# XuyangBai/PointDSC

Measured on AMD Instinct MI355X. Metric: point-cloud pairs/sec @ N=5000 corr, higher is better.
Workload: dtype f32 (attention products as fp16x3 split (fp16 hi+lo operand pairs, three f16 MFMAs per product), f32 accumulate; fc_message / PointCN products as fp16 hi+lo split; spatial-consistency matrix stored as unorm16); 1 GPU; 3DMatch-like synthetic correspondences (BASELINE.json configs[2]): N=5000 corr, 32 pairs per step sharded over 1 GPU(s) = 32 per GPU, 12-layer PointDSC, seeded random weights; num_corr=5000, pairs_per_gpu=32, global_batch=32, compat_format=u16, layer_gemm=h3, att_leaves=canonical, latency_mode=False, range_guard=lazy (pipeline), collective=none (single process, no process group)

## Files before the change

include/pointdsc_hip.h:

```cpp
#ifndef POINTDSC_HIP_H
#define POINTDSC_HIP_H

#include <stddef.h>

#ifdef __cplusplus
extern "C" {
#endif

#define PDSC_VERSION 9
#define PDSC_CHANNELS 128
#define PDSC_MAX_K 64
#define PDSC_MAX_POWER_ITERS 32

enum pdsc_status {
    PDSC_OK = 0,
    PDSC_ERR_ARG = -1,
    PDSC_ERR_WORKSPACE = -2,
    PDSC_ERR_LAUNCH = -3
};

typedef struct pdsc_config {
    int in_dim;
    int num_layers;
    int num_channels;
// ... 98 lines not shown
    float* featB_out;
    float* qkv_out;
    void* q_split;
    void* kv_tiles;
    const void* w1; const float* b1;
    const void* w2; const float* b2;
    const void* w3; const float* b3;
    const void* wp; const float* bp;
    const void* wq; const float* bq;
    const void* wq_split;
    const void* wfrag_tail;
    const void* wfrag_head;
    int gemm_format;
    int io_flags;
    int bs, N;
    int kernel;
} pdsc_layer_call;
int pdsc_layer_run(const pdsc_layer_call* call, void* stream);

size_t    pdsc_wsplit_bytes(const pdsc_config* cfg);
long long pdsc_wsplit_offset(const pdsc_config* cfg, int section, int layer);
int       pdsc_wsplit_build(const pdsc_config* cfg, const float* wpack, void* wsplit, void* stream);
#define PDSC_WS_FRAG_TAIL 100
#define PDSC_WS_FRAG_HEAD 101
#define PDSC_WS_FRAG_TAIL_H3 102
#define PDSC_WS_FRAG_HEAD_H3 103
#define PDSC_WS_FOLD_TAIL_H3 104
#define PDSC_WS_FOLD_HEAD_H3 105
#define PDSC_WS_FOLD_W 106
size_t pdsc_wfrag_fold_tail_bytes(void);
size_t pdsc_wfrag_fold_head_bytes(void);
int pdsc_layer_prefers_block(int bs, int N);
int pdsc_layer_h3_uses_coop(int bs, int N);
size_t pdsc_wfrag_tail_bytes(void);
size_t pdsc_wfrag_head_bytes(void);
int pdsc_wfrag_build_tail(const float* w1, const float* b1, const float* w2, const float* b2, const float* w3,
                          const float* b3, void* out, int gemm_format, void* stream);
int pdsc_wfrag_build_head(const float* wp, const float* bp, const float* wq, const float* bq, void* out,
                          int gemm_format, void* stream);

size_t pdsc_attention_scratch_bytes(int bs, int N, int nsplit);
int    pdsc_attention_default_split(int bs, int N);
int    pdsc_sc_attention(const float* qkv, const float* compat, long long ld, float* msg,
                         void* scratch, size_t scratch_bytes, int bs, int N, int nsplit, void* stream);

size_t pdsc_split_q_bytes(int bs, int N);
size_t pdsc_split_kv_bytes(int bs, int N);
int    pdsc_pack_qkv_split(const float* qkv, void* q_split, void* kv_tiles, int bs, int N, void* stream);
size_t pdsc_attention_split_scratch_bytes(int bs, int N, int nsplit);
int    pdsc_attention_split_default_split(int bs, int N);
int    pdsc_attention_leaf_count(int N);
int    pdsc_attention_leaf_plan(int bs, int N, int leaves_mode, int* nsplit, int* nleaf);
size_t pdsc_attention_leaf_scratch_bytes(int bs, int N, int leaves_mode);
int    pdsc_sc_attention_split(const void* q_split, const void* kv_tiles, const float* compat, long long ld,
                               float* msg, void* scratch, size_t scratch_bytes, int bs, int N, int nsplit,
                               void* stream);
int    pdsc_sc_attention_split_u16(const void* q_split, const void* kv_tiles, const unsigned short* compat_u16, long long ld,
                                   float* msg, void* scratch, size_t scratch_bytes, int bs, int N, int nsplit,
                                   void* stream);

int pdsc_attention_trace(long long* device_buffer);

int pdsc_layer_trace(long long* device_buffer);

int pdsc_classifier_hidden(const float* feat, const float* W1, const float* b1, const float* W2, const float* b2, float* h2,
                           int M, void* stream);
// ... 174 lines not shown
```

pointdsc_amd/_lib.py:

```python
from __future__ import annotations

import ctypes as C
import os
from pathlib import Path

PKG = Path(__file__).resolve().parent
LIB_PATH = Path(os.environ.get("POINTDSC_HIP_LIB", PKG / "libpointdsc_hip.so"))


class PointDSCLibraryError(RuntimeError):
    pass


class PdscConfig(C.Structure):
    _fields_ = [
        ("in_dim", C.c_int), ("num_layers", C.c_int), ("num_channels", C.c_int),
        ("num_iterations", C.c_int), ("k", C.c_int), ("refine_iters", C.c_int),
        ("inlier_threshold", C.c_float), ("nms_radius", C.c_float), ("refine_threshold", C.c_float),
        ("attention_precision", C.c_int), ("compat_format", C.c_int), ("layer_gemm", C.c_int),
        ("att_leaves", C.c_int), ("value_fold", C.c_int),
    ]


W_SECTIONS = [
# ... 6 lines not shown
_cfgp = C.POINTER(PdscConfig)


class PdscLayerCall(C.Structure):
    _fields_ = (
        [(n, _vp) for n in ("msg", "part_o", "part_ml")] + [("nsplit", _i), ("Npad", _i)] +
        [(n, _vp) for n in ("res", "feat_in", "feat_out", "featB_out", "qkv_out", "q_split", "kv_tiles",
                            "w1", "b1", "w2", "b2", "w3", "b3", "wp", "bp", "wq", "bq", "wq_split", "wfrag_tail", "wfrag_head")] +
        [(n, _i) for n in ("gemm_format", "io_flags", "bs", "N", "kernel")])

SIGNATURES = {
    "pdsc_version": (_i, []),
    "pdsc_set_range_report": (_i, [_vp]),
    "pdsc_last_error": (C.c_char_p, []),
    "pdsc_experiments_enabled": (_i, []),
    "pdsc_wpack_floats": (_ll, [_cfgp]),
    "pdsc_wpack_offset": (_ll, [_cfgp, _i, _i]),
    "pdsc_compat_ld": (_ll, [_i]),
    "pdsc_workspace_bytes": (_sz, [_cfgp, _i, _i, _i]),
    "pdsc_workspace_offset": (_ll, [_cfgp, _i, _i, _i, C.c_char_p]),
    "pdsc_spatial_compat": (_i, [_vp, _vp, _vp, _vp, _vp, _ll, _i, _i, _vp]),
    "pdsc_spatial_compat_u16": (_i, [_vp, _vp, _vp, _vp, _ll, _i, _i, _vp]),
    "pdsc_selftest_exact_math": (_i, [_vp, _f, _vp, _vp, _ll, _vp]),
    "pdsc_selftest_mfma_valu_neighbour": (_i, [_vp, _i, _i, _vp]),
    "pdsc_classifier_hidden": (_i, [_vp, _vp, _vp, _vp, _vp, _vp, _i, _vp]),
    "pdsc_linear": (_i, [_vp, _ll, _vp, _vp, _vp, _ll, _vp, _ll, _i, _i, _i, _i, _vp]),
    "pdsc_layer0": (_i, [_vp, _i, _vp, _vp, _vp, _i, _vp]),
    "pdsc_layer_run": (_i, [C.POINTER(PdscLayerCall), _vp]),
    "pdsc_wsplit_bytes": (_sz, [_cfgp]),
    "pdsc_wsplit_offset": (_ll, [_cfgp, _i, _i]),
    "pdsc_wsplit_build": (_i, [_cfgp, _vp, _vp, _vp]),
    "pdsc_layer_prefers_block": (_i, [_i, _i]),
    "pdsc_layer_h3_uses_coop": (_i, [_i, _i]),
    "pdsc_wfrag_tail_bytes": (_sz, []),
    "pdsc_wfrag_head_bytes": (_sz, []),
    "pdsc_wfrag_fold_tail_bytes": (_sz, []),
    "pdsc_wfrag_fold_head_bytes": (_sz, []),
    "pdsc_wfrag_build_tail": (_i, [_vp] * 7 + [_i, _vp]),
    "pdsc_wfrag_build_head": (_i, [_vp] * 5 + [_i, _vp]),
    "pdsc_sc_attention_split_partials": (_i, [_vp, _vp, _vp, _i, _ll, _vp, _sz, _i, _i, _i, _i, _vp]),
    "pdsc_split_q_bytes": (_sz, [_i, _i]),
    "pdsc_split_kv_bytes": (_sz, [_i, _i]),
    "pdsc_pack_qkv_split": (_i, [_vp, _vp, _vp, _i, _i, _vp]),
    "pdsc_attention_split_scratch_bytes": (_sz, [_i, _i, _i]),
    "pdsc_attention_split_default_split": (_i, [_i, _i]),
    "pdsc_attention_leaf_count": (_i, [_i]),
    "pdsc_attention_leaf_plan": (_i, [_i, _i, _i, C.POINTER(C.c_int), C.POINTER(C.c_int)]),
    "pdsc_attention_leaf_scratch_bytes": (_sz, [_i, _i, _i]),
    "pdsc_attention_trace": (_i, [_vp]),
    "pdsc_layer_trace": (_i, [_vp]),
    "pdsc_sc_attention_split": (_i, [_vp, _vp, _vp, _ll, _vp, _vp, _sz, _i, _i, _i, _vp]),
    "pdsc_sc_attention_split_u16": (_i, [_vp, _vp, _vp, _ll, _vp, _vp, _sz, _i, _i, _i, _vp]),
    "pdsc_attention_scratch_bytes": (_sz, [_i, _i, _i]),
    "pdsc_attention_default_split": (_i, [_i, _i]),
    "pdsc_sc_attention": (_i, [_vp, _vp, _ll, _vp, _vp, _sz, _i, _i, _i, _vp]),
    "pdsc_normalize_confidence": (_i, [_vp, _vp, _vp, _vp, _vp, _vp, _i, _vp]),
    "pdsc_nms_keys": (_i, [_vp, _vp, _f, _vp, _i, _i, _vp]),
    "pdsc_nms_workspace_bytes": (_sz, [_i, _i]),
    "pdsc_nms_keys_grid": (_i, [_vp, _vp, _f, _vp, _vp, _sz, _i, _i, _vp]),
    "pdsc_rank_select": (_i, [_vp, _vp, _i, _i, _i, _vp]),
    "pdsc_knn_seeds": (_i, [_vp, _vp, _vp, _vp, _i, _i, _i, _i, _vp]),
    "pdsc_knn_seeds_form": (_i, [_vp, _vp, _vp, _vp, _vp, _i, _i, _i, _i, _i, _vp]),
    "pdsc_normalize_confidence_pf": (_i, [_vp, _vp, _vp, _vp, _vp, _vp, _vp, _i, _i, _vp]),
    "pdsc_seed_power_iteration": (_i, [_vp, _vp, _vp, _vp, _vp, _vp, _vp, _vp, _vp, _i, _i, _i, _i, _i, _vp]),
    "pdsc_seed_solve": (_i, [_vp] * 11 + [_i, _i, _i, _i, _i, _vp]),
    "pdsc_seed_transforms": (_i, [_vp, _vp, _vp, _vp, _vp, _vp, _vp, _i, _i, _i, _i, _i, _vp]),
# ... 86 lines not shown
```

pointdsc_amd/csrc/layer_args.h:

```cpp
#pragma once
#include "pdsc_common.h"
#include "merge_partials.h"

namespace pdsc {

struct LayerArgs {
    const float* msg;
    const float* part_o;
    const float* part_ml;
    int nsplit, Npad;
    const float* res;
    const float* feat_in;
    float* feat_out;
    float* featB_out;
    float* qkv_out;
    const float *w1, *b1, *w2, *b2, *w3, *b3;
    const float *wp, *bp, *wq, *bq;
    const sp16* wq_split;
    sp16* qs;
    unsigned char* kv;
    int N, bs;
    const unsigned char* wf_tail;
    const unsigned char* wf_head;
    int gemm_format;
    int io_flags;
    int stagger_cycles, stagger_mode;
    long long* trace;
    unsigned int* range_flag;
    int value_fold;
    const int* nvalid;
};

enum class LayerKernel { Block, Wave, H3, X3 };
constexpr int layer_merge_limit(LayerKernel k) {
    return k == LayerKernel::Block ? MERGE_MAX_SPLIT_BLOCK : k == LayerKernel::H3 ? MERGE_MAX_SPLIT_H3 : MERGE_MAX_SPLIT;
}

inline LayerArgs layer_args_from_call(const pdsc_layer_call& c) {
    LayerArgs a{};
    a.msg = c.msg; a.part_o = c.part_o; a.part_ml = c.part_ml; a.nsplit = c.nsplit; a.Npad = c.Npad;
    a.res = c.res; a.feat_in = c.feat_in; a.feat_out = c.feat_out; a.featB_out = c.featB_out; a.qkv_out = c.qkv_out;
    a.qs = (sp16*)c.q_split; a.kv = (unsigned char*)c.kv_tiles;
    a.w1 = (const float*)c.w1; a.b1 = c.b1; a.w2 = (const float*)c.w2; a.b2 = c.b2; a.w3 = (const float*)c.w3; a.b3 = c.b3;
    a.wp = (const float*)c.wp; a.bp = c.bp; a.wq = (const float*)c.wq; a.bq = c.bq; a.wq_split = (const sp16*)c.wq_split;
    a.wf_tail = (const unsigned char*)c.wfrag_tail; a.wf_head = (const unsigned char*)c.wfrag_head;
    a.gemm_format = c.gemm_format; a.io_flags = c.io_flags;
    a.N = c.N; a.bs = c.bs;
    return a;
}

int validate_layer_args(const LayerArgs& a, LayerKernel kernel, const char* who);
int dispatch_layer(const LayerArgs& a, LayerKernel kernel, hipStream_t st);

int launch_layer_wave(const LayerArgs& a, bool tail, bool head, hipStream_t st);
int launch_layer_h3(const LayerArgs& a, bool tail, bool head, hipStream_t st);
int launch_layer_h3_coop(const LayerArgs& a, bool tail, bool head, hipStream_t st);
int launch_layer_x3(const LayerArgs& a, bool tail, bool head, hipStream_t st);
bool launch_layer_h3_fits(const LayerArgs& a, bool tail, bool head);
enum class H3Form { TailHeadPF, HeadPF, TailHead, Tail, Head, FoldTailHeadPF, FoldHeadPF, FoldTail, Unserved };
H3Form layer_h3_form(const LayerArgs& a, bool tail, bool head);
int build_value_fold(const float* w1, const float* b1, const float* wqkv, const float* bqkv, const float* w2, const float* b2,
                     const float* w3, const float* b3, const float* wp, const float* bp, float* wfold, void* tail_out, void* head_out,
                     hipStream_t st);
// ... 5 lines not shown
```

pointdsc_amd/csrc/layer_h3.hip:

```cpp
#include <stdlib.h>
#include <type_traits>
#include "pdsc_common.h"
#include "split_layout.h"
#include "merge_partials.h"
#include "layer_args.h"
#include "layer_wave.h"

namespace pdsc {

constexpr int PDSC_H3_COOP_TILES = 2560;

#define LH_STAMP(k) \
    if (TRACE && lane == 0) a.trace[(size_t)gw * 64 + (k)] = __builtin_readcyclecounter();

template <bool F = false>
constexpr int stage_tiles(int stage) { return stage == ST_FC1 || stage == ST_FC2 ? 2 : stage == ST_FC3 || stage == ST_PCN ? 4 : F ? 10 : 12; }

template <bool T, bool H, bool TRACE = false, int PIPE = 6, int EXP = 0, bool FB_PF = false, int NWV = LW_WAVES, int NBUF = 2, bool F = false>
__global__ __launch_bounds__(64 * NWV, NBUF > 2 ? 1 : 2) void layer_h3_kernel(LayerArgs a) {
    __shared__ __attribute__((aligned(16))) float Vs_all[NWV][32 * LW_VLD];
    const int lane = threadIdx.x & 63;
    const int wave = __builtin_amdgcn_readfirstlane(threadIdx.x >> 6);
    const int l31 = lane & 31, h = lane >> 5;
    const int tpp = ceil_div_dev(a.N, 32);
    const int gw = blockIdx.x * NWV + wave;
    if (gw >= a.bs * tpp) return;
    const int b = gw / tpp, tile = gw - b * tpp;
    const int m0 = b * a.N + tile * 32;
    const int valid = min(32, (a.nvalid ? a.nvalid[b] : a.N) - tile * 32);
    if (valid <= 0) return;
    const bool live = l31 < valid;
    const size_t row = (size_t)m0 + min(l31, valid - 1);
    float* Vs = Vs_all[wave];
    unsigned char* patch = reinterpret_cast<unsigned char*>(Vs);

    if (a.stagger_cycles > 0 && blockIdx.x < 512) {
        unsigned hwid;
        asm volatile("s_getreg_b32 %0, hwreg(HW_REG_HW_ID)" : "=s"(hwid));
        const bool late = a.stagger_mode == 1 ? (hwid & 1u) : a.stagger_mode == 2 ? (blockIdx.x & 1) : ((blockIdx.x >> 8) & 1);
        if (late) {
            const long long t0 = __builtin_readcyclecounter();
            while (__builtin_readcyclecounter() - t0 < a.stagger_cycles) __builtin_amdgcn_s_sleep(32);
        }
    }
    LH_STAMP(0)
    float rmax = 0.f;
    constexpr int NCH = num_chunks<T, H, F>();
    constexpr int VW = F ? LW_FOLD_VW : PDSC_CHANNELS;
    constexpr int NQ = VW / 8;
    WChunk w[NBUF];
    static_for<0, NBUF - 1>([&](auto jc) {
        constexpr int j = decltype(jc)::value;
        if constexpr (j < NCH) load_chunk<T, true, true, F>(w[j], a, j, lane);
    });

    u32x4 a0h[8], a0l[8], a1h[4], a1l[4], a2h[4], a2l[4], ayh[8], ayl[8], xqh[8], xql[8];
    f32x4 y3[16];
    if (T) {
        f32x4 x0[16];
        auto first_operand = [&](int kk) __attribute__((always_inline)) {
            if constexpr (F) {
                const float* bpr = reinterpret_cast<const float*>(a.wf_tail + LW_FOLD_BPRIME_BYTES);
#pragma unroll
                for (int u = 0; u < 2; ++u) {
                    const f32x4 bv = *reinterpret_cast<const f32x4*>(bpr + 8 * (2 * kk + u) + 4 * h);
#pragma unroll
                    for (int e = 0; e < 4; ++e) x0[2 * kk + u][e] = fmaxf(x0[2 * kk + u][e] + bv[e], 0.f);
                }
                make_kstep<true>(x0[2 * kk], x0[2 * kk + 1], a1h[kk], a1l[kk], rmax);
            } else {
                make_kstep<true>(x0[2 * kk], x0[2 * kk + 1], a0h[kk], a0l[kk], rmax);
            }
        };
        if (a.msg) {
#pragma unroll
            for (int q = 0; q < NQ; ++q) x0[q] = *reinterpret_cast<const f32x4*>(a.msg + row * VW + 8 * q + 4 * h);
#pragma unroll
            for (int kk = 0; kk < NQ / 2; ++kk) first_operand(kk);
        } else {
            with_split_count<MERGE_MAX_SPLIT_H3>(a.nsplit, [&](auto ns_tag) {
                constexpr int NS = decltype(ns_tag)::value;
                constexpr int GQ = (NS <= 2 ? 16 : NS <= 4 ? 8 : 4) < NQ ? (NS <= 2 ? 16 : NS <= 4 ? 8 : 4) : NQ;
                const size_t slot0 = (size_t)b * NS * a.Npad + (row - (size_t)b * a.N);
                const bool pf = a.io_flags & PDSC_IO_PARTIALS_PF;
                const size_t e0 = pf ? ((size_t)b * NS * a.Npad + (size_t)tile * 32) * VW + lane * 4 : slot0 * VW + 4 * h;
                const int eq = pf ? 256 : 8;
                const MergeWeights<NS> mw = merge_row_weights<NS>(a.part_ml, slot0, (size_t)a.Npad);
#pragma unroll
                for (int q0 = 0; q0 < NQ; q0 += GQ) {
                    f32x4 pv[GQ][NS];
#pragma unroll
                    for (int q = 0; q < GQ; ++q)
#pragma unroll
                        for (int sp = 0; sp < NS; ++sp)
                            pv[q][sp] = (EXP & 4) ? f32x4{1.f, 2.f, 3.f, (float)lane}
                                                  : *reinterpret_cast<const f32x4*>(a.part_o + e0 + (size_t)sp * a.Npad * VW + eq * (q0 + q));
#pragma unroll
                    for (int q = 0; q < GQ; ++q) {
#pragma unroll
                        for (int e = 0; e < 4; ++e) {
                            x0[q0 + q][e] = merge_apply<NS>(pv[q], mw, e);
                            asm volatile("" : "+v"(x0[q0 + q][e]));
                        }
                    }
#pragma unroll
                    for (int kk = q0 / 2; kk < (q0 + GQ) / 2; ++kk) first_operand(kk);
                    __builtin_amdgcn_sched_barrier(0);
                }
            });
        }
    } else {
#pragma unroll
        for (int q = 0; q < 16; ++q) y3[q] = *reinterpret_cast<const f32x4*>(a.feat_in + row * PDSC_CHANNELS + 8 * q + 4 * h);
#pragma unroll
        for (int kk = 0; kk < 8; ++kk) make_kstep<true>(y3[2 * kk], y3[2 * kk + 1], ayh[kk], ayl[kk], rmax);
    }
    LH_STAMP(1)

    unsigned char* img = H ? a.kv + (size_t)gw * SPL_TILE_STRIDE : nullptr;
    f32x16 acc, cross;
    f32x4 vp[4];
    u32x4 ev = {0u, 0u, 0u, 0u};
    float vt[8];

    auto epi = [&](auto stage_c, auto tile_c, auto sc, f32x4 (&v)[4]) {
        constexpr ChunkDesc d = {decltype(stage_c)::value, decltype(tile_c)::value, 0, 0};
        constexpr int s = decltype(sc)::value;
        constexpr int n0 = 32 * d.tile;
        if constexpr (d.stage == ST_FC1 || d.stage == ST_FC2) {
            if constexpr (s < 4) {
#pragma unroll
                for (int e = 0; e < 4; ++e) v[s][e] = fmaxf(v[s][e], 0.f);
                if constexpr (s & 1)
                    make_kstep<true>(v[s - 1], v[s], (d.stage == ST_FC1 ? a1h : a2h)[2 * d.tile + (s >> 1)],
                                     (d.stage == ST_FC1 ? a1l : a2l)[2 * d.tile + (s >> 1)], rmax);
            }
        } else if constexpr (d.stage == ST_FC3) {
            if constexpr (s < 4) {
#pragma unroll
                for (int e = 0; e < 4; ++e) y3[4 * d.tile + s][e] = y3[4 * d.tile + s][e] + v[s][e];
                if constexpr (!H && !(EXP & 2)) *reinterpret_cast<f32x4*>(a.feat_out + row * PDSC_CHANNELS + n0 + 8 * s + 4 * h) = y3[4 * d.tile + s];
                if constexpr (H && (s & 1))
                    make_kstep<true>(y3[4 * d.tile + s - 1], y3[4 * d.tile + s], ayh[2 * d.tile + (s >> 1)], ayl[2 * d.tile + (s >> 1)], rmax);
            }
        } else if constexpr (d.stage == ST_PCN) {
            if constexpr (s < 4) {
#pragma unroll
                for (int e = 0; e < 4; ++e) v[s][e] = fmaxf(v[s][e], 0.f);
                if constexpr (FB_PF) {
                    if constexpr (!(EXP & (2 | 64))) *reinterpret_cast<f32x4*>(a.featB_out + (size_t)gw * PF_TILE_FLOATS + pf_offset_floats(4 * d.tile + s) + lane * 4) = v[s];
                } else
                    patch_put_featB(patch, lane, s, v[s]);
// ... 18 lines not shown
                        if constexpr (!(EXP & (2 | 16))) k_chunk_store(img, lane, 4 * (d.tile - 4) + s, ck);
                        else asm volatile("" :: "v"(ck));
                    }
                } else if constexpr (d.tile < 4) {
                    if constexpr (s < 4) {
                        unsigned hi[2], lo[2];
                        split4(v[s], hi, lo);
                        *reinterpret_cast<u32x4*>(patch + l31 * LW_PROW + 64 * h + 16 * s) = chunk_for_store(hi, lo);
                    }
                    if constexpr (s == 3) wave_lds_sync();
                    if constexpr (s >= 4) {
                        const int pt = 8 * (s - 4) + (lane >> 3), piece = lane & 7;
                        sp16* dst = a.qs + ((size_t)m0 + min(pt, valid - 1)) * SPL_Q_LD + (piece >> 2) * PDSC_CHANNELS + n0 + 8 * (piece & 3);
                        if constexpr (!(EXP & (2 | 8))) *reinterpret_cast<u32x4*>(dst) = ev;
                        else asm volatile("" :: "v"(ev), "v"(dst));
                    }
                    if constexpr (s >= 3 && s < 7) ev = patch_line(patch, lane, s - 3);
                } else {
                    if constexpr (s < 4) vt_put(Vs, lane, s, zero_unless(live, v[s]));
                    if constexpr (s == 3) wave_lds_sync();
                    if constexpr (s == 4 || s == 6) vt_gather(Vs, lane, (s - 4) >> 1, vt);
                    if constexpr (s == 5 || s == 7) {
                        u32x4 ch, cl;
                        vt_split(vt, ch, cl);
                        const int off = vt_offset<VW>(lane, (s - 5) >> 1, 32 * (d.tile - 8));
                        if constexpr (!(EXP & (2 | 32))) vt_store<VW>(img, off, ch, cl);
                        else asm volatile("" :: "v"(ch), "v"(cl), "v"(off));
                    }
                }
            }
        }
    };

    static_for<0, NCH>([&](auto ic) {
        constexpr int i = decltype(ic)::value;
        constexpr ChunkDesc d = chunk_desc<T, F>(i);
        if constexpr (i + NBUF - 1 < NCH && !((EXP & 1) && i >= 1)) load_chunk<T, true, true, F>(w[(i + NBUF - 1) % NBUF], a, i + NBUF - 1, lane);
        if constexpr (T && d.stage == ST_FC2 && d.tile == 0 && !(EXP & 4)) {
            const bool pf = a.io_flags & PDSC_IO_RES_PF;
            const float* r0 = a.res + (pf ? (size_t)gw * PF_TILE_FLOATS + lane * 4 : row * PDSC_CHANNELS + 4 * h);
            const int eq = pf ? 256 : 8;
#pragma unroll
            for (int q = 0; q < 16; ++q) y3[q] = *reinterpret_cast<const f32x4*>(r0 + eq * q);
        }
        const WChunk& wc = w[i % NBUF];
        if constexpr (d.chunk == 0) acc = bias_step(wc);
        constexpr bool pending = d.tile > 0;
        using StageC = std::integral_constant<int, d.stage>;
        using PrevC = std::integral_constant<int, d.tile - 1>;
        static_for<0, 4>([&](auto gc) {
            constexpr int g = decltype(gc)::value;
            if constexpr (d.stage == ST_QKV) {
                const sp16x8 wh = __builtin_bit_cast(sp16x8, wc.v[2 * g]), wl = __builtin_bit_cast(sp16x8, wc.v[2 * g + 1]);
                const sp16x8 bh = __builtin_bit_cast(sp16x8, xqh[4 * d.chunk + g]), bl = __builtin_bit_cast(sp16x8, xql[4 * d.chunk + g]);
                acc = PDSC_MFMA_X3(wl, bh, acc, 0, 0, 0);
                acc = PDSC_MFMA_X3(wh, bl, acc, 0, 0, 0);
                acc = PDSC_MFMA_X3(wh, bh, acc, 0, 0, 0);
            } else {
                const u32x4* oh = d.stage == ST_FC1 ? a0h : d.stage == ST_FC2 ? a1h : d.stage == ST_FC3 ? a2h : ayh;
                const u32x4* ol = d.stage == ST_FC1 ? a0l : d.stage == ST_FC2 ? a1l : d.stage == ST_FC3 ? a2l : ayl;
                const f32x16 zero = {0.f, 0.f, 0.f, 0.f, 0.f, 0.f, 0.f, 0.f, 0.f, 0.f, 0.f, 0.f, 0.f, 0.f, 0.f, 0.f};
                const f16x8 wh = __builtin_bit_cast(f16x8, wc.v[2 * g]), wl = __builtin_bit_cast(f16x8, wc.v[2 * g + 1]);
                const f16x8 bh = __builtin_bit_cast(f16x8, oh[4 * d.chunk + g]), bl = __builtin_bit_cast(f16x8, ol[4 * d.chunk + g]);
                cross = __builtin_amdgcn_mfma_f32_32x32x16_f16(wl, bh, (d.chunk == 0 && g == 0) ? zero : cross, 0, 0, 0);
                acc = __builtin_amdgcn_mfma_f32_32x32x16_f16(wh, bh, acc, 0, 0, 0);
                cross = __builtin_amdgcn_mfma_f32_32x32x16_f16(wh, bl, cross, 0, 0, 0);
            }
            if constexpr (pending) {
                if constexpr (d.nchunks == 2) {
                    epi(StageC{}, PrevC{}, std::integral_constant<int, 4 * d.chunk + g>{}, vp);
                } else {
                    epi(StageC{}, PrevC{}, std::integral_constant<int, 2 * g>{}, vp);
                    epi(StageC{}, PrevC{}, std::integral_constant<int, 2 * g + 1>{}, vp);
                }
            }
        });
        if constexpr (d.chunk == d.nchunks - 1) {
#pragma unroll
            for (int g = 0; g < 4; ++g)
#pragma unroll
                for (int e = 0; e < 4; ++e) vp[g][e] = d.stage != ST_QKV ? fmaf(cross[4 * g + e], H3_INV, acc[4 * g + e]) : acc[4 * g + e];
            if constexpr (d.tile == stage_tiles<F>(d.stage) - 1) {
                static_for<0, 8>([&](auto sc) { epi(StageC{}, std::integral_constant<int, d.tile>{}, sc, vp); });
            }
        }
        if constexpr (PIPE > 0) {
#pragma unroll
            for (int k = 0; k < 13; ++k) {
                __builtin_amdgcn_sched_group_barrier(0x008, 1, 0);
                __builtin_amdgcn_sched_group_barrier(0x002, PIPE, 0);
            }
        }
        LH_STAMP(2 + i)
        __builtin_amdgcn_sched_barrier(0);
    });

    LH_STAMP(63)
    range_report(a.range_flag, b, rmax);
}

bool launch_layer_h3_fits(const LayerArgs& a, bool tail, bool head) {
    if (a.gemm_format != PDSC_LAYER_GEMM_H3) return false;
    if (head && (!a.qs || !a.kv || a.qkv_out)) return false;
    if (tail && head && a.feat_out) return false;
    if (tail && !head && !a.feat_out) return false;
    return a.wf_tail || !tail;
}

H3Form layer_h3_form(const LayerArgs& a, bool tail, bool head) {
    const bool fb_pf = a.io_flags & PDSC_IO_FEATB_PF;
    if (a.value_fold) {
        if (tail && head && fb_pf) return H3Form::FoldTailHeadPF;
        if (head && !tail && fb_pf) return H3Form::FoldHeadPF;
        if (tail && !head) return H3Form::FoldTail;
        set_error("pdsc_layer_run(h3): the folded layer exists with point-fragment featB only");
        return H3Form::Unserved;
    }
    if (head && fb_pf) return tail ? H3Form::TailHeadPF : H3Form::HeadPF;
    return tail && head ? H3Form::TailHead : tail ? H3Form::Tail : H3Form::Head;
}

static void h3_launch_shape(int tiles, int* nwv, int* nbuf) {
    *nwv = LW_WAVES; *nbuf = 2;
    (void)tiles;
#ifdef PDSC_EXPERIMENTS
    const int force = env_int("PDSC_LAYER_H3_SHAPE", 0);
    if (force == 42 || force == 23 || force == 13 || force == 24 || force == 14 || force == 22) { *nwv = force / 10; *nbuf = force % 10; }
#endif
}

int launch_layer_h3(const LayerArgs& a, bool tail, bool head, hipStream_t st) {
    const int waves = a.bs * ceil_div(a.N, 32);
    int nwv, nbuf;
    h3_launch_shape(waves, &nwv, &nbuf);
    if (a.value_fold) { nwv = LW_WAVES; nbuf = 2; }
    const dim3 grid(ceil_div(waves, nwv)), block(64 * nwv);
    const H3Form form = layer_h3_form(a, tail, head);
    if (form == H3Form::Unserved) return PDSC_ERR_ARG;
    const bool timed = tail && head;
    int coop_tiles = PDSC_H3_COOP_TILES;
#ifdef PDSC_EXPERIMENTS
    coop_tiles = env_int("PDSC_LAYER_H3_COOP", coop_tiles);
#endif
    if (waves <= coop_tiles && !a.trace) {
        if (timed) profile_mark_begin(PDSC_PROF_LAYER, st);
        const int rc = launch_layer_h3_coop(a, tail, head, st);
        if (timed) profile_mark_end(PDSC_PROF_LAYER, st);
        return rc;
    }
    if (timed) profile_mark_begin(PDSC_PROF_LAYER, st);
#ifdef PDSC_EXPERIMENTS
#define PDSC_H3_LAUNCH_EXTRA(TT, HH, PF)                                                                                            \
        if (nwv == 1 && nbuf == 4) hipLaunchKernelGGL((layer_h3_kernel<TT, HH, false, 6, 0, PF, 1, 4>), grid, block, 0, st, a);      \
        else if (nwv == 2 && nbuf == 3) hipLaunchKernelGGL((layer_h3_kernel<TT, HH, false, 6, 0, PF, 2, 3>), grid, block, 0, st, a); \
        else if (nwv == 1 && nbuf == 3) hipLaunchKernelGGL((layer_h3_kernel<TT, HH, false, 6, 0, PF, 1, 3>), grid, block, 0, st, a); \
        else if (nwv == 2 && nbuf == 4) hipLaunchKernelGGL((layer_h3_kernel<TT, HH, false, 6, 0, PF, 2, 4>), grid, block, 0, st, a); \
        else if (nwv == 2 && nbuf == 2) hipLaunchKernelGGL((layer_h3_kernel<TT, HH, false, 6, 0, PF, 2, 2>), grid, block, 0, st, a); \
        else
#else
#define PDSC_H3_LAUNCH_EXTRA(TT, HH, PF)
#endif
#define PDSC_H3_LAUNCH(TT, HH, PF)                                                                                                  \
    do {                                                                                                                            \
        PDSC_H3_LAUNCH_EXTRA(TT, HH, PF)                                                                                            \
        hipLaunchKernelGGL((layer_h3_kernel<TT, HH, false, 6, 0, PF>), grid, block, 0, st, a);                                       \
    } while (0)
    switch (form) {
        case H3Form::FoldTailHeadPF: hipLaunchKernelGGL((layer_h3_kernel<true, true, false, 6, 0, true, LW_WAVES, 2, true>), grid, block, 0, st, a); break;
        case H3Form::FoldHeadPF: hipLaunchKernelGGL((layer_h3_kernel<false, true, false, 6, 0, true, LW_WAVES, 2, true>), grid, block, 0, st, a); break;
        case H3Form::FoldTail: hipLaunchKernelGGL((layer_h3_kernel<true, false, false, 6, 0, false, LW_WAVES, 2, true>), grid, block, 0, st, a); break;
        case H3Form::TailHeadPF: {
#ifdef PDSC_LAYER_DIAG
            const int ex = env_int("PDSC_LAYER_H3_EXP", 0);
            if (ex == 1) hipLaunchKernelGGL((layer_h3_kernel<true, true, false, 6, 1, true>), grid, block, 0, st, a);
            else if (ex == 2) hipLaunchKernelGGL((layer_h3_kernel<true, true, false, 6, 2, true>), grid, block, 0, st, a);
            else if (ex == 4) hipLaunchKernelGGL((layer_h3_kernel<true, true, false, 6, 4, true>), grid, block, 0, st, a);
            else if (ex == 7) hipLaunchKernelGGL((layer_h3_kernel<true, true, false, 6, 7, true>), grid, block, 0, st, a);
            else if (ex == 8) hipLaunchKernelGGL((layer_h3_kernel<true, true, false, 6, 8, true>), grid, block, 0, st, a);
            else if (ex == 16) hipLaunchKernelGGL((layer_h3_kernel<true, true, false, 6, 16, true>), grid, block, 0, st, a);
            else if (ex == 32) hipLaunchKernelGGL((layer_h3_kernel<true, true, false, 6, 32, true>), grid, block, 0, st, a);
            else if (ex == 64) hipLaunchKernelGGL((layer_h3_kernel<true, true, false, 6, 64, true>), grid, block, 0, st, a);
            else
#endif
            PDSC_H3_LAUNCH(true, true, true);
            break;
        }
        case H3Form::HeadPF: PDSC_H3_LAUNCH(false, true, true); break;
        case H3Form::TailHead:
#ifdef PDSC_EXPERIMENTS
            if (a.trace) hipLaunchKernelGGL((layer_h3_kernel<true, true, true>), dim3(ceil_div(waves, LW_WAVES)), dim3(64 * LW_WAVES), 0, st, a);
            else
#endif
            PDSC_H3_LAUNCH(true, true, false);
            break;
        case H3Form::Tail: PDSC_H3_LAUNCH(true, false, false); break;
        case H3Form::Head: PDSC_H3_LAUNCH(false, true, false); break;
        case H3Form::Unserved: break;
    }
#undef PDSC_H3_LAUNCH
#undef PDSC_H3_LAUNCH_EXTRA
    if (timed) profile_mark_end(PDSC_PROF_LAYER, st);
    return check_launch("pdsc_layer_run(h3)");
}

}

using namespace pdsc;

extern "C" int pdsc_layer_h3_uses_coop(int bs, int N) {
    if (bs <= 0 || N <= 0) return 0;
    int coop_tiles = PDSC_H3_COOP_TILES;
#ifdef PDSC_EXPERIMENTS
    coop_tiles = env_int("PDSC_LAYER_H3_COOP", coop_tiles);
#endif
    return (long long)bs * ceil_div(N, 32) <= coop_tiles ? 1 : 0;
}
```

pointdsc_amd/csrc/merge_partials.h:

```cpp
#pragma once
#include <type_traits>
#include "pdsc_common.h"

namespace pdsc {

constexpr int MERGE_MAX_SPLIT = 4;
constexpr int MERGE_MAX_SPLIT_BLOCK = 8;
constexpr int MERGE_MAX_SPLIT_H3 = 8;

template <int MAX, class F>
__device__ __forceinline__ void with_split_count(int ns, F&& f) {
    static_assert(MAX == 4 || MAX == 8, "the layer kernels merge up to 4 or up to 8 splits");
    using std::integral_constant;
    if constexpr (MAX == 4) {
        switch (ns) {
            case 1: f(integral_constant<int, 1>{}); break;
            case 2: f(integral_constant<int, 2>{}); break;
            case 3: f(integral_constant<int, 3>{}); break;
            default: f(integral_constant<int, 4>{}); break;
        }
    } else {
        switch (ns) {
            case 1: f(integral_constant<int, 1>{}); break;
            case 2: f(integral_constant<int, 2>{}); break;
            case 3: f(integral_constant<int, 3>{}); break;
            case 4: f(integral_constant<int, 4>{}); break;
            case 5: f(integral_constant<int, 5>{}); break;
            case 6: f(integral_constant<int, 6>{}); break;
            case 7: f(integral_constant<int, 7>{}); break;
            default: f(integral_constant<int, 8>{}); break;
        }
    }
}

template <int NS>
struct MergeWeights {
    float w[NS], rden;
};

template <int NS>
__device__ __forceinline__ MergeWeights<NS> merge_row_weights(const float* __restrict__ part_ml, size_t slot0, size_t sp_stride) {
    MergeWeights<NS> r;
    float ls[NS];
#pragma unroll
    for (int sp = 0; sp < NS; ++sp) {
        const float2 ml = *reinterpret_cast<const float2*>(part_ml + (slot0 + (size_t)sp * sp_stride) * 2);
        r.w[sp] = ml.x; ls[sp] = ml.y;
    }
    float mmax = r.w[0];
#pragma unroll
    for (int sp = 1; sp < NS; ++sp) mmax = fmaxf(mmax, r.w[sp]);
    float den = 0.f;
#pragma unroll
    for (int sp = 0; sp < NS; ++sp) {
        r.w[sp] = __builtin_amdgcn_exp2f(r.w[sp] - mmax);
        den = fmaf(ls[sp], r.w[sp], den);
    }
    r.rden = 1.0f / den;
    return r;
}

template <int NS>
__device__ __forceinline__ float merge_apply(const f32x4 (&pv)[NS], const MergeWeights<NS>& mw, int e) {
    float s = 0.f;
#pragma unroll
    for (int sp = 0; sp < NS; ++sp) s = fmaf(pv[sp][e], mw.w[sp], s);
    return s * mw.rden;
}
template <int NS>
__device__ __forceinline__ f32x4 merge_apply(const f32x4 (&pv)[NS], const MergeWeights<NS>& mw) {
    f32x4 v;
#pragma unroll
    for (int e = 0; e < 4; ++e) v[e] = merge_apply<NS>(pv, mw, e);
    return v;
}

}
```

Measured before the change: 2531 pairs/s.

## Add persistent tile-walking H3 layer kernel with next-tile input prefetch

The H3 layer kernel gains a persistent form: a grid sized to the resident wavefronts (taken from an occupancy query) walks tiles with a stride. While a wave is in the QKV stage it prefetches and merges the next tile's inputs (feature rows or split partials) into LDS slabs, and it reloads the first weight chunk so the next tile can start right away. This is meant to hide the per-tile prologue load latency and the launch/tail costs behind compute. In exchange it uses more LDS and registers, which may lower occupancy, and the control flow becomes more complex. By default it is used in place of the one-tile-per-wave launch whenever the shape matches and the cooperative path is not taken.

```diff
diff --git a/include/pointdsc_hip.h b/include/pointdsc_hip.h
--- a/include/pointdsc_hip.h
+++ b/include/pointdsc_hip.h
@@ -154,6 +154,7 @@
 size_t pdsc_wfrag_fold_head_bytes(void);
 int pdsc_layer_prefers_block(int bs, int N);
 int pdsc_layer_h3_uses_coop(int bs, int N);
+int pdsc_layer_h3_select(int kernel, int walk_waves);
 size_t pdsc_wfrag_tail_bytes(void);
 size_t pdsc_wfrag_head_bytes(void);
 int pdsc_wfrag_build_tail(const float* w1, const float* b1, const float* w2, const float* b2, const float* w3,
diff --git a/pointdsc_amd/_lib.py b/pointdsc_amd/_lib.py
--- a/pointdsc_amd/_lib.py
+++ b/pointdsc_amd/_lib.py
@@ -62,6 +62,7 @@
     "pdsc_wsplit_build": (_i, [_cfgp, _vp, _vp, _vp]),
     "pdsc_layer_prefers_block": (_i, [_i, _i]),
     "pdsc_layer_h3_uses_coop": (_i, [_i, _i]),
+    "pdsc_layer_h3_select": (_i, [_i, _i]),
     "pdsc_wfrag_tail_bytes": (_sz, []),
     "pdsc_wfrag_head_bytes": (_sz, []),
     "pdsc_wfrag_fold_tail_bytes": (_sz, []),
diff --git a/pointdsc_amd/csrc/layer_args.h b/pointdsc_amd/csrc/layer_args.h
--- a/pointdsc_amd/csrc/layer_args.h
+++ b/pointdsc_amd/csrc/layer_args.h
@@ -29,6 +29,7 @@
     unsigned int* range_flag;
     int value_fold;
     const int* nvalid;
+    int pers_waves;
 };
 
 enum class LayerKernel { Block, Wave, H3, X3 };
diff --git a/pointdsc_amd/csrc/layer_h3.hip b/pointdsc_amd/csrc/layer_h3.hip
--- a/pointdsc_amd/csrc/layer_h3.hip
+++ b/pointdsc_amd/csrc/layer_h3.hip
@@ -1,4 +1,5 @@
 #include <stdlib.h>
+#include <atomic>
 #include <type_traits>
 #include "pdsc_common.h"
 #include "split_layout.h"
@@ -16,21 +17,32 @@
 template <bool F = false>
 constexpr int stage_tiles(int stage) { return stage == ST_FC1 || stage == ST_FC2 ? 2 : stage == ST_FC3 || stage == ST_PCN ? 4 : F ? 10 : 12; }
 
-template <bool T, bool H, bool TRACE = false, int PIPE = 6, int EXP = 0, bool FB_PF = false, int NWV = LW_WAVES, int NBUF = 2, bool F = false>
+template <bool T, bool H, bool TRACE = false, int PIPE = 6, int EXP = 0, bool FB_PF = false, int NWV = LW_WAVES, int NBUF = 2, bool F = false,
+          bool PERS = false>
 __global__ __launch_bounds__(64 * NWV, NBUF > 2 ? 1 : 2) void layer_h3_kernel(LayerArgs a) {
+    static_assert(!PERS || (NBUF == 2 && !TRACE), "the two-tile form: product launch shape, no shader-clock trace");
     __shared__ __attribute__((aligned(16))) float Vs_all[NWV][32 * LW_VLD];
-    const int lane = threadIdx.x & 63;
+    int lane = threadIdx.x & 63;
     const int wave = __builtin_amdgcn_readfirstlane(threadIdx.x >> 6);
-    const int l31 = lane & 31, h = lane >> 5;
+    int l31 = lane & 31, h = lane >> 5;
     const int tpp = ceil_div_dev(a.N, 32);
-    const int gw = blockIdx.x * NWV + wave;
-    if (gw >= a.bs * tpp) return;
-    const int b = gw / tpp, tile = gw - b * tpp;
-    const int m0 = b * a.N + tile * 32;
-    const int valid = min(32, (a.nvalid ? a.nvalid[b] : a.N) - tile * 32);
+    const int ntiles = a.bs * tpp;
+    int gw = blockIdx.x * NWV + wave;
+    const int gstep = PERS ? a.pers_waves : 0;
+    if (gw >= (PERS ? min(gstep, ntiles) : ntiles)) return;
+    auto tile_rows = [&](int g) { const int bb = g / tpp; return min(32, (a.nvalid ? a.nvalid[bb] : a.N) - (g - bb * tpp) * 32); };
+    if constexpr (PERS) {
+        while (tile_rows(gw) <= 0) {
+            gw += gstep;
+            if (gw >= ntiles) return;
+        }
+    }
+    int b = gw / tpp, tile = gw - b * tpp;
+    int m0 = b * a.N + tile * 32;
+    int valid = min(32, (a.nvalid ? a.nvalid[b] : a.N) - tile * 32);
     if (valid <= 0) return;
-    const bool live = l31 < valid;
-    const size_t row = (size_t)m0 + min(l31, valid - 1);
+    bool live = l31 < valid;
+    size_t row = (size_t)m0 + min(l31, valid - 1);
     float* Vs = Vs_all[wave];
     unsigned char* patch = reinterpret_cast<unsigned char*>(Vs);
 
@@ -56,38 +68,158 @@
 
     u32x4 a0h[8], a0l[8], a1h[4], a1l[4], a2h[4], a2l[4], ayh[8], ayl[8], xqh[8], xql[8];
     f32x4 y3[16];
-    if (T) {
+    LayerArgs aw = a;
+    auto operand_of = [&](f32x4& xa, f32x4& xb, int kk, u32x4& oh, u32x4& ol, float& rm) __attribute__((always_inline)) {
+        if constexpr (F) {
+            const float* bpr = reinterpret_cast<const float*>(aw.wf_tail + LW_FOLD_BPRIME_BYTES);
+            const f32x4 ba = *reinterpret_cast<const f32x4*>(bpr + 8 * (2 * kk) + 4 * h);
+            const f32x4 bb = *reinterpret_cast<const f32x4*>(bpr + 8 * (2 * kk + 1) + 4 * h);
+#pragma unroll
+            for (int e = 0; e < 4; ++e) xa[e] = fmaxf(xa[e] + ba[e], 0.f);
+#pragma unroll
+            for (int e = 0; e < 4; ++e) xb[e] = fmaxf(xb[e] + bb[e], 0.f);
+        }
+        make_kstep<true>(xa, xb, oh, ol, rm);
+    };
+    u32x4* const in_h = !T ? ayh : F ? a1h : a0h;
+    u32x4* const in_l = !T ? ayl : F ? a1l : a0l;
+
+    constexpr int PF_REGS = 4, PF_MAX_NS = 4, PF_PIECES = 8;
+    constexpr int QCH = 2 * stage_tiles<F>(ST_QKV);
+    __shared__ u32x4 Nx_all[PERS ? NWV : 1][PERS ? PF_PIECES : 1][64];
+    u32x4 (*Nx)[64] = Nx_all[PERS ? wave : 0];
+    f32x4 pfb[PERS ? PF_REGS : 1];
+    f32x4 pcarry = {0.f, 0.f, 0.f, 0.f};
+    float2 pml[PERS ? PF_MAX_NS : 1];
+    __shared__ float Nw_all[PERS ? NWV : 1][PERS ? PF_MAX_NS + 1 : 1][64];
+    float (*Nw)[64] = Nw_all[PERS ? wave : 0];
+    const float* pbase = nullptr;
+    float rmaxN = 0.f;
+    int gwN = ntiles;
+    bool pre = false;
+    constexpr bool PF_FORM = H && (!T || FB_PF);
+    const bool pf_can = PF_FORM && (T ? (!a.msg && a.nsplit >= 1 && a.nsplit <= PF_MAX_NS) : true);
+    auto slab_put = [&](f32x4& xa, f32x4& xb, int kk) __attribute__((always_inline)) {
+        u32x4 oh, ol;
+        if constexpr (T) operand_of(xa, xb, kk, oh, ol, rmaxN);
+        else make_kstep<true>(xa, xb, oh, ol, rmaxN);
+        Nx[2 * kk][lane] = oh;
+        Nx[2 * kk + 1][lane] = ol;
+    };
+    auto prefetch_step = [&](auto cc) __attribute__((always_inline)) {
+        constexpr int c = decltype(cc)::value;
+        if constexpr (!T) {
+            constexpr int S = (QCH - 2) / 3;
+            if constexpr (c % S == 0 && c / S <= 2) {
+                constexpr int k = c / S;
+                if constexpr (k >= 1) {
+                    slab_put(pfb[0], pfb[1], 2 * (k - 1));
+                    slab_put(pfb[2], pfb[3], 2 * (k - 1) + 1);
+                }
+                if constexpr (k < 2) {
+                    if constexpr (k == 0) {
+                        const int bN = gwN / tpp, tN = gwN - bN * tpp;
+                        const int vN = min(32, (a.nvalid ? a.nvalid[bN] : a.N) - tN * 32);
+                        pbase = a.feat_in + ((size_t)bN * a.N + tN * 32 + min(l31, vN - 1)) * PDSC_CHANNELS + 4 * h;
+                    }
+#pragma unroll
+                    for (int q = 0; q < 4; ++q) pfb[q] = *reinterpret_cast<const f32x4*>(pbase + 8 * (4 * k + q));
+                }
+                __builtin_amdgcn_sched_barrier(0);
+            }
+        } else {
+            with_split_count<MERGE_MAX_SPLIT>(a.nsplit, [&](auto ns_tag) __attribute__((always_inline)) {
+                constexpr int NS = decltype(ns_tag)::value;
+                static_assert(NS <= PF_MAX_NS && MERGE_MAX_SPLIT == PF_MAX_NS, "one piece of every split fits the batch registers");
+                constexpr int GQ = PF_REGS / NS;
+                constexpr int NB = PF_PIECES / GQ;
+                constexpr int S = (QCH - 2) / (NB + 1);
+                if constexpr (c % S == 0 && c / S <= NB) {
+                    constexpr int k = c / S;
+                    const int eq = (a.io_flags & PDSC_IO_PARTIALS_PF) ? 256 : 8;
+                    const size_t sps = (size_t)a.Npad * VW;
+                    if constexpr (k >= 1) {
+                        MergeWeights<NS> mw;
+                        if constexpr (k == 1) {
+                            float2 ml[NS];
+#pragma unroll
+                            for (int sp = 0; sp < NS; ++sp) ml[sp] = pml[sp];
+                            mw = merge_weights_of<NS>(ml);
+#pragma unroll
+                            for (int sp = 0; sp < NS; ++sp) Nw[sp][lane] = mw.w[sp];
+                            Nw[PF_MAX_NS][lane] = mw.rden;
+                        } else {
+#pragma unroll
+                            for (int sp = 0; sp < NS; ++sp) mw.w[sp] = Nw[sp][lane];
+                            mw.rden = Nw[PF_MAX_NS][lane];
+                        }
+                        f32x4 xm[GQ];
+#pragma unroll
+                        for (int q = 0; q < GQ; ++q) {
+                            f32x4 pv[NS];
+#pragma unroll
+                            for (int sp = 0; sp < NS; ++sp) pv[sp] = pfb[q * NS + sp];
+#pragma unroll
+                            for (int e = 0; e < 4; ++e) {
+                                xm[q][e] = merge_apply<NS>(pv, mw, e);
+                                asm volatile("" : "+v"(xm[q][e]));
+                            }
+                        }
+                        if constexpr (GQ == 1) {
+                            if constexpr ((k - 1) % 2 == 0) pcarry = xm[0];
+                            else slab_put(pcarry, xm[0], (k - 1) / 2);
+                        } else {
+#pragma unroll
+                            for (int j = 0; j < GQ / 2; ++j) slab_put(xm[2 * j], xm[2 * j + 1], ((k - 1) * GQ) / 2 + j);
+                        }
+                    }
+                    if constexpr (k < NB) {
+                        if constexpr (k == 0) {
+                            const int bN = gwN / tpp, tN = gwN - bN * tpp;
+                            const int vN = min(32, (a.nvalid ? a.nvalid[bN] : a.N) - tN * 32);
+                            const size_t slot0 = (size_t)bN * NS * a.Npad + (size_t)(tN * 32 + min(l31, vN - 1));
+                            pbase = a.part_o + ((a.io_flags & PDSC_IO_PARTIALS_PF) ? ((size_t)bN * NS * a.Npad + (size_t)tN * 32) * VW + lane * 4
+                                                                                     : slot0 * VW + 4 * h);
+#pragma unroll
+                            for (int sp = 0; sp < NS; ++sp)
+                                pml[sp] = *reinterpret_cast<const float2*>(a.part_ml + (slot0 + (size_t)sp * a.Npad) * 2);
+                        }
+#pragma unroll
+                        for (int q = 0; q < GQ; ++q)
+#pragma unroll
+                            for (int sp = 0; sp < NS; ++sp)
+                                pfb[q * NS + sp] = (EXP & 4) ? f32x4{1.f, 2.f, 3.f, (float)lane}
+                                                             : *reinterpret_cast<const f32x4*>(pbase + sp * sps + eq * (k * GQ + q));
+                    }
+                    __builtin_amdgcn_sched_barrier(0);
+                }
+            });
+        }
+    };
+
+    auto prologue = [&](auto start_c) __attribute__((always_inline)) {
+    constexpr int START = decltype(start_c)::value;
+    if constexpr (T) {
         f32x4 x0[16];
-        auto first_operand = [&](int kk) __attribute__((always_inline)) {
-            if constexpr (F) {
-                const float* bpr = reinterpret_cast<const float*>(a.wf_tail + LW_FOLD_BPRIME_BYTES);
-#pragma unroll
-                for (int u = 0; u < 2; ++u) {
-                    const f32x4 bv = *reinterpret_cast<const f32x4*>(bpr + 8 * (2 * kk + u) + 4 * h);
-#pragma unroll
-                    for (int e = 0; e < 4; ++e) x0[2 * kk + u][e] = fmaxf(x0[2 * kk + u][e] + bv[e], 0.f);
-                }
-                make_kstep<true>(x0[2 * kk], x0[2 * kk + 1], a1h[kk], a1l[kk], rmax);
-            } else {
-                make_kstep<true>(x0[2 * kk], x0[2 * kk + 1], a0h[kk], a0l[kk], rmax);
-            }
-        };
+        auto first_operand = [&](int kk) __attribute__((always_inline)) { operand_of(x0[2 * kk], x0[2 * kk + 1], kk, in_h[kk], in_l[kk], rmax); };
         if (a.msg) {
 #pragma unroll
-            for (int q = 0; q < NQ; ++q) x0[q] = *reinterpret_cast<const f32x4*>(a.msg + row * VW + 8 * q + 4 * h);
-#pragma unroll
-            for (int kk = 0; kk < NQ / 2; ++kk) first_operand(kk);
+            for (int q = START; q < NQ; ++q) x0[q] = *reinterpret_cast<const f32x4*>(a.msg + row * VW + 8 * q + 4 * h);
+#pragma unroll
+            for (int kk = START / 2; kk < NQ / 2; ++kk) first_operand(kk);
         } else {
             with_split_count<MERGE_MAX_SPLIT_H3>(a.nsplit, [&](auto ns_tag) {
                 constexpr int NS = decltype(ns_tag)::value;
-                constexpr int GQ = (NS <= 2 ? 16 : NS <= 4 ? 8 : 4) < NQ ? (NS <= 2 ? 16 : NS <= 4 ? 8 : 4) : NQ;
+                constexpr int GQB = (NS <= 2 ? 16 : NS <= 4 ? 8 : 4) / (PERS ? 2 : 1);
+                constexpr int GQ0 = GQB < NQ ? GQB : NQ;
+                constexpr int GQ = GQ0 < NQ - START ? GQ0 : NQ - START;
                 const size_t slot0 = (size_t)b * NS * a.Npad + (row - (size_t)b * a.N);
                 const bool pf = a.io_flags & PDSC_IO_PARTIALS_PF;
                 const size_t e0 = pf ? ((size_t)b * NS * a.Npad + (size_t)tile * 32) * VW + lane * 4 : slot0 * VW + 4 * h;
                 const int eq = pf ? 256 : 8;
                 const MergeWeights<NS> mw = merge_row_weights<NS>(a.part_ml, slot0, (size_t)a.Npad);
 #pragma unroll
-                for (int q0 = 0; q0 < NQ; q0 += GQ) {
+                for (int q0 = START; q0 < NQ; q0 += GQ) {
                     f32x4 pv[GQ][NS];
 #pragma unroll
                     for (int q = 0; q < GQ; ++q)
@@ -111,13 +243,13 @@
         }
     } else {
 #pragma unroll
-        for (int q = 0; q < 16; ++q) y3[q] = *reinterpret_cast<const f32x4*>(a.feat_in + row * PDSC_CHANNELS + 8 * q + 4 * h);
-#pragma unroll
-        for (int kk = 0; kk < 8; ++kk) make_kstep<true>(y3[2 * kk], y3[2 * kk + 1], ayh[kk], ayl[kk], rmax);
-    }
-    LH_STAMP(1)
-
-    unsigned char* img = H ? a.kv + (size_t)gw * SPL_TILE_STRIDE : nullptr;
+        for (int q = START; q < 16; ++q) y3[q] = *reinterpret_cast<const f32x4*>(a.feat_in + row * PDSC_CHANNELS + 8 * q + 4 * h);
+#pragma unroll
+        for (int kk = START / 2; kk < 8; ++kk) make_kstep<true>(y3[2 * kk], y3[2 * kk + 1], ayh[kk], ayl[kk], rmax);
+    }
+    };
+
+    unsigned char* img = nullptr;
     f32x16 acc, cross;
     f32x4 vp[4];
     u32x4 ev = {0u, 0u, 0u, 0u};
@@ -202,10 +334,37 @@
         }
     };
 
+    for (;;) {
+    if constexpr (PERS) {
+        asm volatile("" : "+s"(aw.wf_tail), "+s"(aw.wf_head), "+v"(lane));
+        l31 = lane & 31; h = lane >> 5;
+        gwN = gw + gstep;
+        while (gwN < ntiles && tile_rows(gwN) <= 0) gwN += gstep;
+        bool in_line = true;
+        if constexpr (PF_FORM) {
+            if (pre) {
+                in_line = false;
+#pragma unroll
+                for (int kk = 0; kk < PF_PIECES / 2; ++kk) { in_h[kk] = Nx[2 * kk][lane]; in_l[kk] = Nx[2 * kk + 1][lane]; }
+                if constexpr (!T || !F) prologue(std::integral_constant<int, PF_PIECES>{});
+            }
+        }
+        if (in_line) prologue(std::integral_constant<int, 0>{});
+    } else {
+        prologue(std::integral_constant<int, 0>{});
+    }
+    LH_STAMP(1)
+    img = H ? a.kv + (size_t)gw * SPL_TILE_STRIDE : nullptr;
+    const bool pf_now = PERS && pf_can && gwN < ntiles;
+
     static_for<0, NCH>([&](auto ic) {
         constexpr int i = decltype(ic)::value;
         constexpr ChunkDesc d = chunk_desc<T, F>(i);
-        if constexpr (i + NBUF - 1 < NCH && !((EXP & 1) && i >= 1)) load_chunk<T, true, true, F>(w[(i + NBUF - 1) % NBUF], a, i + NBUF - 1, lane);
+        if constexpr (i + NBUF - 1 < NCH && !((EXP & 1) && i >= 1)) load_chunk<T, true, true, F>(w[(i + NBUF - 1) % NBUF], aw, i + NBUF - 1, lane);
+        if constexpr (PERS && i == NCH - 1 && !(EXP & 1)) load_chunk<T, true, true, F>(w[0], aw, 0, lane);
+        if constexpr (PERS && PF_FORM && d.stage == ST_QKV) {
+            if (pf_now) prefetch_step(std::integral_constant<int, 2 * d.tile + d.chunk>{});
+        }
         if constexpr (T && d.stage == ST_FC2 && d.tile == 0 && !(EXP & 4)) {
             const bool pf = a.io_flags & PDSC_IO_RES_PF;
             const float* r0 = a.res + (pf ? (size_t)gw * PF_TILE_FLOATS + lane * 4 : row * PDSC_CHANNELS + 4 * h);
@@ -267,6 +426,20 @@
 
     LH_STAMP(63)
     range_report(a.range_flag, b, rmax);
+    if constexpr (!PERS) {
+        break;
+    } else {
+        if (gwN >= ntiles) break;
+        gw = gwN;
+        b = gw / tpp; tile = gw - b * tpp;
+        m0 = b * a.N + tile * 32;
+        valid = min(32, (a.nvalid ? a.nvalid[b] : a.N) - tile * 32);
+        live = l31 < valid;
+        row = (size_t)m0 + min(l31, valid - 1);
+        pre = pf_now;
+        rmax = rmaxN; rmaxN = 0.f;
+    }
+    }
 }
 
 bool launch_layer_h3_fits(const LayerArgs& a, bool tail, bool head) {
@@ -299,12 +472,30 @@
 #endif
 }
 
-int launch_layer_h3(const LayerArgs& a, bool tail, bool head, hipStream_t st) {
+static std::atomic<int> g_h3_kernel{0}, g_h3_walk_waves{0};
+
+template <class K>
+static int h3_resident_waves(K kernel, int nwv, int slot) {
+    static std::atomic<int> cache[16][12];
+    int dev = 0;
+    if (hipGetDevice(&dev) != hipSuccess || dev < 0 || dev >= 16) dev = 0;
+    int waves = cache[dev][slot].load(std::memory_order_relaxed);
+    if (waves > 0) return waves;
+    int per_cu = 0, cus = 0;
+    if (hipOccupancyMaxActiveBlocksPerMultiprocessor(&per_cu, kernel, 64 * nwv, 0) != hipSuccess || per_cu <= 0) return 0;
+    if (hipDeviceGetAttribute(&cus, hipDeviceAttributeMultiprocessorCount, dev) != hipSuccess || cus <= 0) return 0;
+    waves = per_cu * cus * nwv;
+    cache[dev][slot].store(waves, std::memory_order_relaxed);
+    return waves;
+}
+
+int launch_layer_h3(const LayerArgs& a_in, bool tail, bool head, hipStream_t st) {
+    LayerArgs a = a_in;
     const int waves = a.bs * ceil_div(a.N, 32);
     int nwv, nbuf;
     h3_launch_shape(waves, &nwv, &nbuf);
     if (a.value_fold) { nwv = LW_WAVES; nbuf = 2; }
-    const dim3 grid(ceil_div(waves, nwv)), block(64 * nwv);
+    dim3 grid(ceil_div(waves, nwv)), block(64 * nwv);
     const H3Form form = layer_h3_form(a, tail, head);
     if (form == H3Form::Unserved) return PDSC_ERR_ARG;
     const bool timed = tail && head;
@@ -312,12 +503,17 @@
 #ifdef PDSC_EXPERIMENTS
     coop_tiles = env_int("PDSC_LAYER_H3_COOP", coop_tiles);
 #endif
-    if (waves <= coop_tiles && !a.trace) {
+    const int sel = g_h3_kernel.load(std::memory_order_relaxed);
+    if (sel == 0 && waves <= coop_tiles && !a.trace) {
         if (timed) profile_mark_begin(PDSC_PROF_LAYER, st);
         const int rc = launch_layer_h3_coop(a, tail, head, st);
         if (timed) profile_mark_end(PDSC_PROF_LAYER, st);
         return rc;
     }
+    bool two = sel != 1 && !a.trace && nwv == LW_WAVES && nbuf == 2;
+#ifdef PDSC_EXPERIMENTS
+    two = two && env_int("PDSC_LAYER_H3_TWO_TILE", 1) != 0;
+#endif
     if (timed) profile_mark_begin(PDSC_PROF_LAYER, st);
 #ifdef PDSC_EXPERIMENTS
 #define PDSC_H3_LAUNCH_EXTRA(TT, HH, PF)                                                                                            \
@@ -335,6 +531,41 @@
         PDSC_H3_LAUNCH_EXTRA(TT, HH, PF)                                                                                            \
         hipLaunchKernelGGL((layer_h3_kernel<TT, HH, false, 6, 0, PF>), grid, block, 0, st, a);                                       \
     } while (0)
+    if (two) {
+#define PDSC_H3_WALK(SLOT, ...)                                                                                                     \
+    do {                                                                                                                            \
+        const int forced = g_h3_walk_waves.load(std::memory_order_relaxed);                                                         \
+        const int res = forced > 0 ? forced : h3_resident_waves(layer_h3_kernel<__VA_ARGS__>, LW_WAVES, SLOT);                      \
+        if (res <= 0) { set_error("pdsc_layer_run(h3): occupancy query of the two-tile kernel failed"); return PDSC_ERR_LAUNCH; }  \
+        a.pers_waves = res < waves ? res : waves;                                                                                   \
+        grid = dim3(ceil_div(a.pers_waves, LW_WAVES));                                                                              \
+        hipLaunchKernelGGL((layer_h3_kernel<__VA_ARGS__>), grid, block, 0, st, a);                                                  \
+    } while (0)
+        switch (form) {
+            case H3Form::FoldTailHeadPF: PDSC_H3_WALK(0, true, true, false, 6, 0, true, LW_WAVES, 2, true, true); break;
+            case H3Form::FoldHeadPF: PDSC_H3_WALK(1, false, true, false, 6, 0, true, LW_WAVES, 2, true, true); break;
+            case H3Form::FoldTail: PDSC_H3_WALK(2, true, false, false, 6, 0, false, LW_WAVES, 2, true, true); break;
+            case H3Form::TailHeadPF: {
+#ifdef PDSC_LAYER_DIAG
+                const int ex = env_int("PDSC_LAYER_H3_EXP", 0);
+                if (ex == 2) PDSC_H3_WALK(8, true, true, false, 6, 2, true, LW_WAVES, 2, false, true);
+                else if (ex == 4) PDSC_H3_WALK(9, true, true, false, 6, 4, true, LW_WAVES, 2, false, true);
+                else if (ex == 7) PDSC_H3_WALK(10, true, true, false, 6, 7, true, LW_WAVES, 2, false, true);
+                else
+#endif
+                PDSC_H3_WALK(3, true, true, false, 6, 0, true, LW_WAVES, 2, false, true);
+                break;
+            }
+            case H3Form::HeadPF: PDSC_H3_WALK(4, false, true, false, 6, 0, true, LW_WAVES, 2, false, true); break;
+            case H3Form::TailHead: PDSC_H3_WALK(5, true, true, false, 6, 0, false, LW_WAVES, 2, false, true); break;
+            case H3Form::Tail: PDSC_H3_WALK(6, true, false, false, 6, 0, false, LW_WAVES, 2, false, true); break;
+            case H3Form::Head: PDSC_H3_WALK(7, false, true, false, 6, 0, false, LW_WAVES, 2, false, true); break;
+            case H3Form::Unserved: break;
+        }
+#undef PDSC_H3_WALK
+        if (timed) profile_mark_end(PDSC_PROF_LAYER, st);
+        return check_launch("pdsc_layer_run(h3)");
+    }
     switch (form) {
         case H3Form::FoldTailHeadPF: hipLaunchKernelGGL((layer_h3_kernel<true, true, false, 6, 0, true, LW_WAVES, 2, true>), grid, block, 0, st, a); break;
         case H3Form::FoldHeadPF: hipLaunchKernelGGL((layer_h3_kernel<false, true, false, 6, 0, true, LW_WAVES, 2, true>), grid, block, 0, st, a); break;
@@ -377,8 +608,16 @@
 
 using namespace pdsc;
 
+extern "C" int pdsc_layer_h3_select(int kernel, int walk_waves) {
+    PDSC_REQUIRE(kernel >= 0 && kernel <= 2 && walk_waves >= 0, "pdsc_layer_h3_select: kernel=%d (0 by tile count, 1 one tile per wavefront, "
+                 "2 two-tile walk), walk_waves=%d (0 = the resident wavefronts)", kernel, walk_waves);
+    g_h3_kernel.store(kernel);
+    g_h3_walk_waves.store(walk_waves);
+    return PDSC_OK;
+}
+
 extern "C" int pdsc_layer_h3_uses_coop(int bs, int N) {
-    if (bs <= 0 || N <= 0) return 0;
+    if (bs <= 0 || N <= 0 || g_h3_kernel.load() != 0) return 0;
     int coop_tiles = PDSC_H3_COOP_TILES;
 #ifdef PDSC_EXPERIMENTS
     coop_tiles = env_int("PDSC_LAYER_H3_COOP", coop_tiles);
diff --git a/pointdsc_amd/csrc/merge_partials.h b/pointdsc_amd/csrc/merge_partials.h
--- a/pointdsc_amd/csrc/merge_partials.h
+++ b/pointdsc_amd/csrc/merge_partials.h
@@ -39,14 +39,11 @@
 };
 
 template <int NS>
-__device__ __forceinline__ MergeWeights<NS> merge_row_weights(const float* __restrict__ part_ml, size_t slot0, size_t sp_stride) {
+__device__ __forceinline__ MergeWeights<NS> merge_weights_of(const float2 (&ml)[NS]) {
     MergeWeights<NS> r;
     float ls[NS];
 #pragma unroll
-    for (int sp = 0; sp < NS; ++sp) {
-        const float2 ml = *reinterpret_cast<const float2*>(part_ml + (slot0 + (size_t)sp * sp_stride) * 2);
-        r.w[sp] = ml.x; ls[sp] = ml.y;
-    }
+    for (int sp = 0; sp < NS; ++sp) { r.w[sp] = ml[sp].x; ls[sp] = ml[sp].y; }
     float mmax = r.w[0];
 #pragma unroll
     for (int sp = 1; sp < NS; ++sp) mmax = fmaxf(mmax, r.w[sp]);
@@ -58,6 +55,14 @@
     }
     r.rden = 1.0f / den;
     return r;
+}
+
+template <int NS>
+__device__ __forceinline__ MergeWeights<NS> merge_row_weights(const float* __restrict__ part_ml, size_t slot0, size_t sp_stride) {
+    float2 ml[NS];
+#pragma unroll
+    for (int sp = 0; sp < NS; ++sp) ml[sp] = *reinterpret_cast<const float2*>(part_ml + (slot0 + (size_t)sp * sp_stride) * 2);
+    return merge_weights_of<NS>(ml);
 }
 
 template <int NS>
```

New measurement: 2500 pairs/s. 1.2% lower.
